# ziwang1121/IEEE

Measured on AMD Instinct MI355X. Metric: 3-modal images/s (train fwd+bwd), higher is better.
Workload: dtype bf16

## Files before the change

### ieee_amd/csrc/bn.hip

```cpp
#include <math.h>
#include <stdlib.h>

#include <hip/hip_ext.h>

#include <algorithm>
#include "common.h"
#include "pool_gather.h"

namespace ieee {

#ifndef IEEE_RED_MAX_BLOCKS
#define IEEE_RED_MAX_BLOCKS 768
#endif
constexpr int RED_MAX_BLOCKS = IEEE_RED_MAX_BLOCKS;

struct RedGeom {
  int M, C;
  int cprw;
  int tx, ty;
  int cblocks;
  int rblocks;
  int rows_per_block;
};

// ... 369 lines not shown
      const float* sp = stats + z * stats_gs + 2 * C + c0;
      load_floats<VEC>(sp, sc);
      load_floats<VEC>(sp + C, sh);
    }
  }
  const T* dd = da + z * gs;
  const T* aa = MASK == 1 ? a + z * gs : nullptr;
  const T* yy = y + z * gs;
  T* oo = dy + z * gs;
  T* go = GOUT ? gout + z * gs : nullptr;
  const int64_t stride = (int64_t)gridDim.x * 256;
  auto finish = [&](int64_t i, const uint4& dv, const uint4& yv, const uint4& av) {
    float d[VEC], v[VEC], m[VEC];
    Vec16<T>::unpack(dv, d);
    Vec16<T>::unpack(yv, v);
    if (MASK == 1) {
      Vec16<T>::unpack(av, m);
#pragma unroll
      for (int e = 0; e < VEC; ++e) d[e] = m[e] > 0.f ? d[e] : 0.f;
    } else if (MASK == 2) {
#pragma unroll
      for (int e = 0; e < VEC; ++e) d[e] = (v[e] * sc[e] + sh[e]) > 0.f ? d[e] : 0.f;
    }
    if (GOUT) *(uint4*)(go + i * VEC) = Vec16<T>::pack(d);
#pragma unroll
    for (int e = 0; e < VEC; ++e) v[e] = k1[e] * d[e] + k2[e] * v[e] + k3[e];
    *(uint4*)(oo + i * VEC) = Vec16<T>::pack(v);
  };
  int64_t i = (int64_t)blockIdx.x * 256 + threadIdx.x;
  if (UNROLL == 2)
    for (; i + stride < total_chunks; i += 2 * stride) {
      const int64_t j = i + stride;
      const uint4 d0 = *(const uint4*)(dd + i * VEC), d1 = *(const uint4*)(dd + j * VEC);
      const uint4 y0 = *(const uint4*)(yy + i * VEC), y1 = *(const uint4*)(yy + j * VEC);
      uint4 a0 = y0, a1 = y1;
      if (MASK == 1) { a0 = *(const uint4*)(aa + i * VEC); a1 = *(const uint4*)(aa + j * VEC); }
      finish(i, d0, y0, a0);
      finish(j, d1, y1, a1);
    }
  for (; i < total_chunks; i += stride) {
    const uint4 d0 = *(const uint4*)(dd + i * VEC);
    const uint4 y0 = *(const uint4*)(yy + i * VEC);
    uint4 a0 = y0;
    if (MASK == 1) a0 = *(const uint4*)(aa + i * VEC);
    finish(i, d0, y0, a0);
  }
}

constexpr double TOT_INV_FWD = 1.0 / 16777216.0;
constexpr double TOT_INV_BWD = 1.0 / 1099511627776.0;
constexpr long long TOT_HALF_RANGE = 1ll << 61;
__device__ __forceinline__ long long tot_abs(long long v) { return v < 0 ? -v : v; }

template <typename T, bool RES, bool BITS>
__global__ __launch_bounds__(256) void bn_apply_totals_kernel(const T* __restrict__ y, const T* __restrict__ residual,
                                                              T* __restrict__ out, const long long* __restrict__ totals,
                                                              const float* __restrict__ gamma, const float* __restrict__ beta,
                                                              int64_t param_gs, float* running_mean, float* running_var,
                                                              int64_t buf_gs, float* __restrict__ stats, int M, float momentum,
                                                              float eps, int64_t total_chunks, int cprw, int C, int64_t gs,
                                                              int relu, uint8_t* __restrict__ relu_bits, double inv_m,
                                                              float unbias, int rep, int64_t rep_stride, int* overflow) {
  constexpr int VEC = 16 / sizeof(T);
  const int z = blockIdx.y;
  uint8_t* bb = BITS ? relu_bits + z * (gs / 8) : nullptr;
  const int c0 = (threadIdx.x & (cprw - 1)) * VEC;
  const T* yy = y + z * gs;
  const T* rr = RES ? residual + z * gs : nullptr;
  const int64_t stride = (int64_t)gridDim.x * 256;
  int64_t i = (int64_t)blockIdx.x * 256 + threadIdx.x;
  uint4 ynext = make_uint4(0, 0, 0, 0), rnext = make_uint4(0, 0, 0, 0);
  if (out != nullptr && i < total_chunks) {
    ynext = *(const uint4*)(yy + i * VEC);
    if (RES) rnext = *(const uint4*)(rr + i * VEC);
  }
  extern __shared__ float tot_lds[];
  float* s_sc = tot_lds;
  float* s_sh = tot_lds + C;
  for (int c = threadIdx.x; c < C; c += 256) {
    long long t1 = 0, t2 = 0;
    for (int r = 0; r < rep; ++r) {
      t1 += totals[r * rep_stride + (int64_t)z * 2 * C + c];
      t2 += totals[r * rep_stride + (int64_t)z * 2 * C + C + c];
    }
    if (blockIdx.x == 0 && overflow != nullptr && (tot_abs(t1) > TOT_HALF_RANGE || tot_abs(t2) > TOT_HALF_RANGE)) *(volatile int*)(overflow + 2) = 1;
    const float ga = gamma[z * param_gs + c], be = beta[z * param_gs + c];
    const double mu = (double)t1 * inv_m;
    double var = (double)t2 * inv_m - mu * mu;
    if (var < 0) var = 0;
    const float mean = (float)mu, varf = (float)var, invstd = rsqrtf(varf + eps);
    const float scv = ga * invstd, shv = be - mean * scv;
    s_sc[c] = scv; s_sh[c] = shv;
    if (blockIdx.x == 0) {
      float* st = stats + (int64_t)z * 4 * C;
      st[c] = mean; st[C + c] = invstd; st[2 * C + c] = scv; st[3 * C + c] = shv;
      if (running_mean != nullptr) {
        float* rm = running_mean + z * buf_gs + c;
        float* rv = running_var + z * buf_gs + c;
        *rm = (1.f - momentum) * *rm + momentum * mean;
        *rv = (1.f - momentum) * *rv + momentum * (varf * unbias);
      }
    }
  }
  __syncthreads();
  float sc[VEC], sh[VEC];
  load_floats<VEC>(s_sc + c0, sc);
  load_floats<VEC>(s_sh + c0, sh);
  if (out == nullptr) return;
  T* oo = out + z * gs;
  for (; i < total_chunks; i += stride) {
    float v[VEC], r[VEC];
    Vec16<T>::unpack(ynext, v);
    if (RES) Vec16<T>::unpack(rnext, r);
    if (i + stride < total_chunks) {
      ynext = *(const uint4*)(yy + (i + stride) * VEC);
      if (RES) rnext = *(const uint4*)(rr + (i + stride) * VEC);
    }
#pragma unroll
    for (int e = 0; e < VEC; ++e) {
      float x = v[e] * sc[e] + sh[e];
      if (RES) x += r[e];
      if (relu) x = fmaxf(x, 0.f);
      v[e] = x;
    }
    const uint4 pv = Vec16<T>::pack(v);
    *(uint4*)(oo + i * VEC) = pv;
    if constexpr (BITS && VEC == 8) {
      Vec16<T>::unpack(pv, v);
      unsigned b = 0;
#pragma unroll
      for (int e = 0; e < VEC; ++e) b |= (v[e] > 0.f ? 1u : 0u) << e;
      bb[i] = (uint8_t)b;
    }
  }
}

template <typename T, int MASK, bool GOUT>
__global__ __launch_bounds__(256) void bn_bwd_apply_totals_kernel(const T* __restrict__ da, const T* __restrict__ a,
                                                                  const T* __restrict__ y, T* __restrict__ dy,
                                                                  T* __restrict__ gout, const long long* __restrict__ totals,
                                                                  const float* __restrict__ gamma, int64_t param_gs,
                                                                  const float* __restrict__ stats, float* dgamma,
                                                                  float* dbeta, int64_t grad_gs, int M, int64_t total_chunks,
                                                                  int cprw, int C, int64_t gs, double inv_m, int rep,
                                                                  int64_t rep_stride, int* overflow) {
  constexpr int VEC = 16 / sizeof(T);
  const int z = blockIdx.y;
  const int c0 = (threadIdx.x & (cprw - 1)) * VEC;
  const float* st = stats + (int64_t)z * 4 * C;
  const T* dd = da + z * gs;
  const T* aa = MASK == 1 ? a + z * gs : nullptr;
  const T* yy = y + z * gs;
  const int64_t stride = (int64_t)gridDim.x * 256;
  int64_t i = (int64_t)blockIdx.x * 256 + threadIdx.x;
  uint4 dnext = make_uint4(0, 0, 0, 0), ynext = dnext, anext = dnext;
  if (i < total_chunks) {
    dnext = *(const uint4*)(dd + i * VEC);
    ynext = *(const uint4*)(yy + i * VEC);
    if (MASK == 1) anext = *(const uint4*)(aa + i * VEC);
  }
  extern __shared__ float tot_lds[];
  float* s_k = tot_lds;
  for (int c = threadIdx.x; c < C; c += 256) {
    long long t1 = 0, t2 = 0;
    for (int r = 0; r < rep; ++r) {
      t1 += totals[r * rep_stride + (int64_t)z * 2 * C + c];
      t2 += totals[r * rep_stride + (int64_t)z * 2 * C + C + c];
    }
    if (blockIdx.x == 0 && overflow != nullptr && (tot_abs(t1) > TOT_HALF_RANGE || tot_abs(t2) > TOT_HALF_RANGE)) *(volatile int*)(overflow + 3) = 1;
// ... 557 lines not shown

namespace ieee {
__global__ void bn_frozen_coef_kernel(const float* __restrict__ stats, int64_t stats_gs, float* __restrict__ coef,
                                      int64_t coef_gs, int C) {
  const int c = blockIdx.x * blockDim.x + threadIdx.x;
  if (c >= C) return;
  float* k = coef + blockIdx.y * coef_gs;
  k[c] = stats[blockIdx.y * stats_gs + 2 * C + c];
  k[C + c] = 0.f;
  k[2 * C + c] = 0.f;
}
}

extern "C" int ieee_bn2d_bwd_frozen(const void* dout, const void* out_mask, const void* y, void* dy, void* g_out, int dtype,
                                    int64_t groups, int64_t M, int64_t C, int64_t act_gs, const float* stats, float* coef,
                                    int mask_from_y, void* done_event, void* stream) {
  IEEE_REQUIRE(dout && y && dy && stats && coef, "bn2d_bwd_frozen: null pointer");
  IEEE_REQUIRE(dtype == IEEE_F32 || dtype == IEEE_BF16, "bn2d_bwd_frozen: bad dtype");
  IEEE_REQUIRE(C % vec_of(dtype) == 0, "bn2d_bwd_frozen: C not a multiple of the vector width");
  hipStream_t st = (hipStream_t)stream;
  bn_frozen_coef_kernel<<<dim3(cdiv(C, 256), (unsigned)groups), 256, 0, st>>>(stats, 4 * C, coef, 3 * C, (int)C);
  IEEE_TRY(launch_status("bn_frozen_coef_kernel"));
  return launch_bwd_apply(dout, out_mask, y, dy, g_out, dtype, groups, M, C, act_gs, stats, coef, mask_from_y, done_event, st);
}

extern "C" int ieee_bn2d_fwd_totals(const void* y, const void* residual, void* out, int dtype, int64_t groups, int64_t M,
                                    int64_t C, int64_t act_gs, const float* gamma, const float* beta, int64_t param_gs,
                                    float* running_mean, float* running_var, int64_t buf_gs, float* stats, const void* totals,
                                    int replicas, float momentum, float eps, int relu, void* relu_bits, int* overflow,
                                    void* stream) {
  IEEE_REQUIRE(replicas >= 1 && replicas <= 64, "bn2d_fwd_totals: 1..64 replicas");
  IEEE_REQUIRE(y && gamma && beta && stats && totals, "bn2d_fwd_totals: null pointer");
  IEEE_REQUIRE(dtype == IEEE_BF16, "bn2d_fwd_totals: bf16 only (the fused statistics exist on the bf16 path)");
  const int cprw = (int)(C / 8);
  IEEE_REQUIRE(C % 8 == 0 && cprw >= 1 && cprw <= 256 && 256 % cprw == 0, "bn2d_fwd_totals: C / 8 must divide 256");
  IEEE_REQUIRE(!relu_bits || (out && act_gs % 8 == 0), "bn2d_fwd_totals: relu_bits needs an output");
  IEEE_REQUIRE((((uintptr_t)totals | (uintptr_t)gamma | (uintptr_t)beta) & 15) == 0 && param_gs % 4 == 0,
               "bn2d_fwd_totals: totals / gamma / beta must be 16-byte aligned (group stride a multiple of 4 floats)");
  hipStream_t st = (hipStream_t)stream;
  const int64_t chunks = M * C / 8;
  dim3 grid(out ? tot_blocks(chunks, groups) : 1, (unsigned)groups);
  const bf16 *yb = (const bf16*)y, *rb = (const bf16*)residual;
  bf16* ob = (bf16*)out;
  uint8_t* bits = (uint8_t*)relu_bits;
#define IEEE_BN_TOT(RES, BITS)                                                                                              \
  bn_apply_totals_kernel<bf16, RES, BITS><<<grid, 256, 2 * C * sizeof(float), st>>>(yb, rb, ob, (const long long*)totals, gamma, beta, param_gs, \
      running_mean, running_var, buf_gs, stats, (int)M, momentum, eps, chunks, cprw, (int)C, act_gs, relu, bits,       \
      TOT_INV_FWD / (double)M, M > 1 ? (float)((double)M / (double)(M - 1)) : 1.0f, replicas, groups * 2 * C, overflow)
  if (residual && bits) IEEE_BN_TOT(true, true);
  else if (residual) IEEE_BN_TOT(true, false);
  else if (bits) IEEE_BN_TOT(false, true);
  else IEEE_BN_TOT(false, false);
#undef IEEE_BN_TOT
  return launch_status("bn_apply_totals_kernel");
}

extern "C" int ieee_bn2d_bwd_totals(const void* dout, const void* out_mask, const void* y, void* dy, void* g_out, int dtype,
                                    int64_t groups, int64_t M, int64_t C, int64_t act_gs, const float* gamma,
                                    int64_t param_gs, const float* stats, float* dgamma, float* dbeta, int64_t grad_gs,
                                    const void* totals, int replicas, int mask_from_y, int* overflow, void* done_event,
                                    void* stream) {
  IEEE_REQUIRE(replicas >= 1 && replicas <= 64, "bn2d_bwd_totals: 1..64 replicas");
  IEEE_REQUIRE(dout && y && dy && gamma && stats && totals, "bn2d_bwd_totals: null pointer");
  IEEE_REQUIRE(dtype == IEEE_BF16, "bn2d_bwd_totals: bf16 only");
  const int cprw = (int)(C / 8);
  IEEE_REQUIRE(C % 8 == 0 && cprw >= 1 && cprw <= 256 && 256 % cprw == 0, "bn2d_bwd_totals: C / 8 must divide 256");
  IEEE_REQUIRE((((uintptr_t)totals | (uintptr_t)gamma | (uintptr_t)stats) & 15) == 0 && param_gs % 4 == 0,
               "bn2d_bwd_totals: totals / gamma / stats must be 16-byte aligned (group stride a multiple of 4 floats)");
  hipStream_t st = (hipStream_t)stream;
  hipEvent_t ev = (hipEvent_t)done_event;
  const int64_t chunks = M * C / 8;
  dim3 grid(tot_blocks(chunks, groups), (unsigned)groups);
  const int variant = (out_mask ? 1 : (mask_from_y ? 2 : 0)) * 2 + (g_out ? 1 : 0);
#define IEEE_BN_BWD_TOT(MASK, GOUT)                                                                                          \
  case MASK * 2 + (GOUT ? 1 : 0):                                                                                            \
    hipExtLaunchKernelGGL((bn_bwd_apply_totals_kernel<bf16, MASK, GOUT>), grid, dim3(256), 3 * C * sizeof(float), st,        \
                          nullptr, ev, 0,                                                                                    \
                          (const bf16*)dout, (const bf16*)out_mask, (const bf16*)y, (bf16*)dy, (bf16*)g_out,                 \
                          (const long long*)totals, gamma, param_gs, stats, dgamma, dbeta, grad_gs, (int)M, chunks, cprw,    \
                          (int)C, act_gs, 1.0 / (double)M, replicas, groups * 2 * C, overflow);                              \
    break;
  switch (variant) {
    IEEE_BN_BWD_TOT(0, false) IEEE_BN_BWD_TOT(0, true) IEEE_BN_BWD_TOT(1, false) IEEE_BN_BWD_TOT(1, true)
    IEEE_BN_BWD_TOT(2, false) IEEE_BN_BWD_TOT(2, true)
  }
#undef IEEE_BN_BWD_TOT
  return launch_status("bn_bwd_apply_totals_kernel");
}

extern "C" int ieee_bn2d_bwd_totals_ds(const void* dout, const void* y, const void* y_ds, void* dy, int dtype, int64_t groups,
                                       int64_t M, int64_t C, int64_t act_gs, const float* gamma, int64_t param_gs,
                                       const float* stats, float* dgamma, float* dbeta, int64_t grad_gs, const void* totals,
                                       int replicas, void* totals_ds, int replicas_ds, int* overflow, void* done_event,
                                       void* stream) {
  IEEE_REQUIRE(replicas >= 1 && replicas <= 64 && replicas_ds >= 1 && replicas_ds <= 64, "bn2d_bwd_totals_ds: 1..64 replicas");
  IEEE_REQUIRE(dout && y && y_ds && dy && gamma && stats && totals && totals_ds, "bn2d_bwd_totals_ds: null pointer");
  IEEE_REQUIRE(dtype == IEEE_BF16, "bn2d_bwd_totals_ds: bf16 only");
  const int cprw = (int)(C / 8);
  IEEE_REQUIRE(C % 8 == 0 && cprw >= 1 && cprw <= 256 && 256 % cprw == 0, "bn2d_bwd_totals_ds: C / 8 must divide 256");
  IEEE_REQUIRE((((uintptr_t)totals | (uintptr_t)gamma | (uintptr_t)stats) & 15) == 0 && param_gs % 4 == 0,
               "bn2d_bwd_totals_ds: totals / gamma / stats must be 16-byte aligned (group stride a multiple of 4 floats)");
  hipStream_t st = (hipStream_t)stream;
  const int64_t chunks = M * C / 8;
  dim3 grid(tot_blocks(chunks, groups), (unsigned)groups);
  const size_t lds = std::max<size_t>(3 * C, 8 * 256) * sizeof(float);
  const float lim2 = nextafterf(4611686018427387904.0f / (float)grid.x, 0.f);
// ... 82 lines not shown
```

### ieee_amd/csrc/net.hip

```cpp
#include <stdio.h>
#include <stdlib.h>
#include <string.h>

#include <map>
#include <string>
#include <vector>

#include "common.h"

namespace {

using namespace ieee;

struct Tensor {
  size_t off = 0;
  int64_t numel = 0;
  int dtype = IEEE_F32;
};

static constexpr int TOT_REP_MAX = 8;
static int totals_tiles() {
  static const int t = getenv("IEEE_BN_TOTALS_TILES") ? atoi(getenv("IEEE_BN_TOTALS_TILES")) : 1024;
  return t;
}
// ... 49 lines not shown
  return m;
}

struct Block {
  int c1, c2, c3, ds;
};

struct Net {
  static constexpr int NGBUF = 15;
  int B, H, W, num_classes, dtype, interaction, attention, using_rem;
  int frozen = 0;
  int parts = 6, rdim = 768, cdim = 128, fdim = 2048, hid = 128;
  float bn_eps = 1e-5f, bn_mom = 0.1f;
  std::vector<std::string> slot_names;
  std::vector<int64_t> slot_off;
  std::vector<int> triples;
  float *params = nullptr, *grads = nullptr, *buffers = nullptr;
  bool bound = false;
  std::vector<ConvUnit> units;
  std::vector<Block> blocks;
  int u_stem = -1, u_one = -1, u_rest = -1;
  int s_ca1, s_ca2, s_rw, s_rg, s_rb, s_rrm, s_rrv, s_rem_param, s_rem_pw, s_rem_pb, s_rem_qw, s_rem_qb;
  int s_fcw[18], s_fcb[18], s_fcg[18], s_fcbe[18], s_fcrm[18], s_fcrv[18], s_clw[18], s_clb[18];
  size_t ws_bytes = 0;
  std::map<std::string, Tensor> tensors;
  Tensor x0, pool, pool_arg, S, gbuf[NGBUF], slab, bnpart, bncoef, bnpart2, bncoef2, packtab, gemm_work;
  static constexpr int RT_SLOTS = 24, RT_MAX = 32;
  Tensor rtab;
  std::vector<ieee_wgrad_reduce_desc> rpend;
  std::vector<ieee_wgrad_reduce_desc> rtab_host[RT_SLOTS];
  const void* rtab_ws[RT_SLOTS] = {};
  ConvUnit reduce_unit;
  size_t tot_begin = 0, tot_end = 0;
  Tensor slab2;
  ieee_wgrad_reduce_desc wpend = {};
  int wflip = 0;
  Tensor wtickets;
  Tensor tickets;
  std::vector<PackDescHost> pack_train, pack_eval;
  int pack_blocks_train = 0, pack_blocks_eval = 0;
  std::vector<PackDescHost> pack_late;
  int pack_late_first = 0, pack_late_unit = 0, pack_blocks_early = 0, pack_blocks_late = 0;
  std::vector<PackDescHost> pack_train_s, pack_late_s;
  int pack_blocks_train_s = 0, pack_late_first_s = 0, pack_blocks_early_s = 0, pack_blocks_late_s = 0;
  const void* shadow = nullptr;
  hipEvent_t pack_ev[2] = {nullptr, nullptr};
  const void* pack_uploaded_ws = nullptr;
  bool fused_bwd_state = false;
  Tensor oflags;
  const void* last_ws = nullptr;
  bool totals_off = false;
  bool bwd_totals_fresh = false;
  bool bwd_totals_state = false;
  bool stem_a_valid = false;
  bool eval_cache_valid = false;
  const void* eval_cache_ws = nullptr;
  hipStream_t side = nullptr;
  hipStream_t side2 = nullptr;
  hipEvent_t branch_ev[16] = {};
  std::vector<hipEvent_t> side_ready;
  hipEvent_t gbuf_read[NGBUF] = {};
  hipEvent_t side_done = nullptr;
  hipEvent_t sync_ev = nullptr;
  bool gbuf_pending[NGBUF] = {};
  uint64_t gbuf_seq[NGBUF] = {}, gbuf_clock = 0;
  int gbuf_evt[NGBUF] = {};
  bool side_dirty = false;
  size_t side_used = 0;
  ~Net() {
    for (hipEvent_t e : ev_pool) (void)hipEventDestroy(e);
    for (hipEvent_t e : side_ready) (void)hipEventDestroy(e);
    for (hipEvent_t e : gbuf_read) if (e) (void)hipEventDestroy(e);
    if (side_done) (void)hipEventDestroy(side_done);
    if (sync_ev) (void)hipEventDestroy(sync_ev);
    for (hipEvent_t e : pack_ev) if (e) (void)hipEventDestroy(e);
    if (side) (void)hipStreamDestroy(side);
    for (hipEvent_t e : branch_ev) if (e) (void)hipEventDestroy(e);
    if (side2) (void)hipStreamDestroy(side2);
  }
  Tensor Gp, avgmax, amax, Hh, Hs, att, Pp, Zg, Zp, glob, part, sv_g, sv_p, rr, part2, fcraw, sv_fc, featcat, fcall,
      logits, featn, norms;
  Tensor dfeatcat, dfcraw, dpart2, dr, dglob, dZp, dZg, dPp, dGp, datt, dHs, dH, davgmax, remwork;
  int esz() const { return dtype == IEEE_BF16 ? 2 : 4; }
  char* tap_base = nullptr;
  size_t tap_bytes = 0, tap_used = 0;
  std::map<std::string, Tensor> taps;
  int profiling = 0;
  std::vector<hipEvent_t> ev_pool;
  std::vector<int> ev_cat;
  std::vector<std::string> ev_name;
  std::vector<const char*> ev_label;
  std::vector<double> ev_flops;
  size_t ev_used = 0;
  double prof_flops[2] = {0, 0};
  int64_t prof_launches[2] = {0, 0};

  int slot3(const std::string& pattern) {
    const int id = (int)slot_names.size();
    triples.push_back(id);
    for (int m = 0; m < 3; ++m) {
      std::string s = pattern;
      const size_t p = s.find("{m}");
      s.replace(p, 3, std::to_string(m));
      slot_names.push_back(s);
    }
    return id;
// ... 277 lines not shown
    Tensor t;
    t.off = n.tap_used; t.numel = numel; t.dtype = dt;
    IEEE_HIP(hipMemcpyAsync(n.tap_base + t.off, p, bytes, hipMemcpyDeviceToDevice, (hipStream_t)st));
    n.taps[name] = t;
    n.tap_used += (bytes + 255) / 256 * 256;
    return IEEE_OK;
  }
  int64_t in_numel(const ConvUnit& u) const { return (int64_t)3 * B * u.Hi * u.Wi * u.Ci; }
  int64_t out_numel(const ConvUnit& u) const { return (int64_t)3 * u.M(B) * u.Co; }
  bool fused_stats = false;
  bool fused_fin = false;
  bool frz(const ConvUnit& u) const { return (n.frozen & u.child) != 0; }
  int totals_rep(const ConvUnit& u) const { return n.totals_off ? 0 : totals_rep_for((u.M(B) + 127) / 128); }
  bool use_totals(const ConvUnit& u) const {
    return n.dtype == IEEE_BF16 && totals_rep(u) > 0 && u.Co % 8 == 0 && 256 % (u.Co / 8) == 0 && u.Co / 8 <= 256 &&
           &u != &n.units[n.u_stem] && ((n.slot_off[u.s_g] | n.slot_off[u.s_b] | gs(u.s_g)) & 3) == 0;
  }
  bool fwd_totals = false;
  int conv(const ConvUnit& u, const void* in, bool want_stats = false) {
    const int64_t ldf = ieee_conv_packed_ld(n.dtype, u.Ci, u.R, u.S);
    fused_stats = want_stats && n.dtype == IEEE_BF16 && !frz(u);
    fwd_totals = fused_stats && use_totals(u);
    static const bool f_fin = getenv("IEEE_BN_FIN_FUSE") && atoi(getenv("IEEE_BN_FIN_FUSE")) != 0;
    fused_fin = f_fin && fused_stats && !fwd_totals && u.M(B) <= ieee_conv2d_fwd_bn_train_max_rows() && u.Ci % 64 == 0 && u.Co % 8 == 0;
    prof_begin(0, u, nullptr, !fused_fin);
    struct G { Run* r; ~G() { r->prof_end(); } } guard{this};
    if (fused_fin)
      return ieee_conv2d_fwd_bn_train(in, P(u.wf), P(u.y), n.dtype, 3, B, u.Hi, u.Wi, u.Ci, u.Co, u.R, u.S, u.stride, u.pad,
                                      (int64_t)B * u.Hi * u.Wi * u.Ci, u.Co * ldf, u.M(B) * u.Co, bnpart_cur, par(u.s_g), par(u.s_b),
                                      gs(u.s_g), buf(u.s_rm), buf(u.s_rv), gs(u.s_rm), F(u.stats), n.bn_mom, n.bn_eps, tickets_cur, st);
    const bool sh = use_shadow && u.shadow_ok;
    const void* wf = sh ? (const void*)((const uint16_t*)n.shadow + n.slot_off[u.s_w]) : P(u.wf);
    return ieee_conv2d_fwd_ex(in, wf, P(u.y), n.dtype, 3, B, u.Hi, u.Wi, u.Ci, u.Co, u.R, u.S, u.stride, u.pad,
                              (int64_t)B * u.Hi * u.Wi * u.Ci, sh ? gs(u.s_w) : u.Co * ldf, u.M(B) * u.Co, fused_stats ? bnpart_cur : nullptr,
                              take_extras(fwd_totals ? P(u.tot_f) : nullptr, (int64_t)2 * u.Co, fwd_totals ? totals_rep(u) : 1), st);
  }
  int bn(const ConvUnit& u, const void* residual, void* out, int relu, int training, void* relu_bits = nullptr) {
    if (frz(u)) training = 0;
    if (training && fwd_totals) {
      fwd_totals = fused_stats = fused_fin = false;
      return ieee_bn2d_fwd_totals(P(u.y), residual, out, n.dtype, 3, u.M(B), u.Co, u.M(B) * u.Co, par(u.s_g), par(u.s_b), gs(u.s_g),
                                  buf(u.s_rm), buf(u.s_rv), gs(u.s_rm), F(u.stats), P(u.tot_f), totals_rep(u), n.bn_mom, n.bn_eps, relu, relu_bits,
                                  oflags_ptr(), st);
    }
    fwd_totals = false;
    const int64_t rb = (training && fused_fin) ? -1 : ((training && fused_stats) ? ieee_conv2d_fwd_stats_rblocks(B, u.Ho, u.Wo) : 0);
    fused_stats = false;
    fused_fin = false;
    if (rb < 0 && out == nullptr) return IEEE_OK;
    return ieee_bn2d_fwd(P(u.y), residual, out, n.dtype, 3, u.M(B), u.Co, u.M(B) * u.Co, par(u.s_g), par(u.s_b),
                         gs(u.s_g), buf(u.s_rm), buf(u.s_rv), gs(u.s_rm), F(u.stats), bnpart_cur, n.bn_mom, n.bn_eps,
                         training, relu, rb, relu_bits, st);
  }
  bool eval_cached = false;
  int conv_bn_eval(const ConvUnit& u, const void* in, const void* residual, void* out, int relu) {
    const int64_t ldf = ieee_conv_packed_ld(n.dtype, u.Ci, u.R, u.S);
    if (!eval_cached)
      IEEE_TRY(ieee_bn2d_fwd(P(u.y), nullptr, nullptr, n.dtype, 3, u.M(B), u.Co, u.M(B) * u.Co, par(u.s_g), par(u.s_b),
                           gs(u.s_g), buf(u.s_rm), buf(u.s_rv), gs(u.s_rm), F(u.stats), bnpart_cur, n.bn_mom, n.bn_eps,
                           0, relu, 0, nullptr, st));
    prof_begin(0, u);
    struct G { Run* r; ~G() { r->prof_end(); } } guard{this};
    return ieee_conv2d_fwd_bn_eval(in, P(u.wf), out, residual, F(u.stats), relu, n.dtype, 3, B, u.Hi, u.Wi, u.Ci, u.Co,
                                   u.R, u.S, u.stride, u.pad, (int64_t)B * u.Hi * u.Wi * u.Ci, u.Co * ldf, u.M(B) * u.Co, st);
  }
  bool& fused_bwd = n.fused_bwd_state;
  hipEvent_t bn_done = nullptr;
  hipEvent_t next_ready_event() {
    if (n.side_used == n.side_ready.size()) {
      hipEvent_t e;
      if (hipEventCreateWithFlags(&e, hipEventDisableTiming) != hipSuccess) return nullptr;
      n.side_ready.push_back(e);
    }
    return n.side_ready[n.side_used++];
  }
  const ConvUnit* ds_pending = nullptr;
  const ConvUnit* ds_totals_ready = nullptr;
  int bn_bwd(const ConvUnit& u, const void* dout, const void* mask, void* dy, void* gout, int mask_from_y = 0,
             float* partial = nullptr, int64_t partial_rb = 0) {
    const int64_t rb = partial ? partial_rb : (fused_bwd ? (u.M(B) + 127) / 128 : 0);
    const bool ds_ready = !partial && ds_totals_ready == &u;
    if (ds_ready) ds_totals_ready = nullptr;
    const bool from_totals = (!partial && fused_bwd && n.bwd_totals_state) || ds_ready;
    const ConvUnit* ds = ds_pending;
    ds_pending = nullptr;
    if (!partial) partial = bnpart_cur;
    fused_bwd = false;
    n.bwd_totals_state = false;
    will_write(dy);
    if (gout) will_write(gout);
    static const bool ride_wanted = !(getenv("IEEE_EVENT_RIDE") && atoi(getenv("IEEE_EVENT_RIDE")) == 0);
    const bool ride = ride_wanted && side_enabled() && ieee_event_ride_selfcheck(st, (void*)n.side) == 0;
    bn_done = ride ? next_ready_event() : nullptr;
    if (frz(u))
      return ieee_bn2d_bwd_frozen(dout, mask, P(u.y), dy, gout, n.dtype, 3, u.M(B), u.Co, u.M(B) * u.Co, F(u.stats), bncoef_cur,
                                  mask_from_y, (void*)bn_done, st);
    if (from_totals && ds != nullptr && mask == nullptr && gout == nullptr && !mask_from_y && use_totals(*ds) && !frz(*ds) && ds->Co == u.Co &&
        ds->M(B) == u.M(B)) {
      ds_totals_ready = ds;
      return ieee_bn2d_bwd_totals_ds(dout, P(u.y), P(ds->y), dy, n.dtype, 3, u.M(B), u.Co, u.M(B) * u.Co, par(u.s_g), gs(u.s_g), F(u.stats),
                                     grd(u.s_g), grd(u.s_b), gs(u.s_g), P(u.tot_b), totals_rep(u), P(ds->tot_b), totals_rep(*ds),
                                     oflags_ptr(), (void*)bn_done, st);
    }
    if (from_totals)
      return ieee_bn2d_bwd_totals(dout, mask, P(u.y), dy, gout, n.dtype, 3, u.M(B), u.Co, u.M(B) * u.Co, par(u.s_g), gs(u.s_g),
                                  F(u.stats), grd(u.s_g), grd(u.s_b), gs(u.s_g), P(u.tot_b), totals_rep(u), mask_from_y, oflags_ptr(),
// ... 317 lines not shown
    const int64_t n_early = use_shadow ? N.pack_late_first_s : N.pack_late_first;
    const int b_train = use_shadow ? N.pack_blocks_train_s : N.pack_blocks_train, b_late = use_shadow ? N.pack_blocks_late_s : N.pack_blocks_late,
              b_early = use_shadow ? N.pack_blocks_early_s : N.pack_blocks_early;
    static const bool pack_async = !(getenv("IEEE_PACK_ASYNC") && atoi(getenv("IEEE_PACK_ASYNC")) == 0);
    if (training && pack_async && side_enabled() && n_late > 0) {
      IEEE_HIP(hipEventRecord(N.pack_ev[0], (hipStream_t)st));
      IEEE_HIP(hipStreamWaitEvent(N.side, N.pack_ev[0], 0));
      IEEE_TRY(ieee_pack_all_weights(N.params, ws, t_late, n_late, b_late, dt, (void*)N.side));
      IEEE_HIP(hipEventRecord(N.pack_ev[1], N.side));
      late_pack_pending = true;
      if (n_early > 0) IEEE_TRY(ieee_pack_all_weights(N.params, ws, t_train, n_early, b_early, dt, st));
    } else if (training)
      IEEE_TRY(ieee_pack_all_weights(N.params, ws, t_train, n_train, b_train, dt, st));
    else if (!(eval_cached = (N.eval_cache_valid && N.eval_cache_ws == (const void*)ws && !N.profiling)))
      IEEE_TRY(ieee_pack_all_weights(N.params, ws, tab_dev, (int64_t)N.pack_eval.size(), N.pack_blocks_eval, dt, st));
    if (training) N.eval_cache_valid = false;
  }
  {
    static const bool f_fin = getenv("IEEE_BN_FIN_FUSE") && atoi(getenv("IEEE_BN_FIN_FUSE")) != 0;
    if (training && f_fin) IEEE_HIP(hipMemsetAsync(P(N.tickets), 0, 512 * 4, (hipStream_t)st));
  }
  if (training && dt == IEEE_BF16 && (totals_tiles() > 0 || wgrad_fold())) {
    IEEE_HIP(hipMemsetAsync(ws + N.tot_begin, 0, N.tot_end - N.tot_begin, (hipStream_t)st));
    N.bwd_totals_fresh = true;
  }
  IEEE_TRY(ieee_nchw_to_nhwc3(xr, xn, xt, P(N.x0), dt, B, 3, N.H, N.W, 4, 3, st));
  const ConvUnit& s = N.units[N.u_stem];
  static const bool fuse_eval = !(getenv("IEEE_EVAL_FUSE") && atoi(getenv("IEEE_EVAL_FUSE")) == 0);
  const bool fe = !training && fuse_eval;
  bool stem_pool_fused = false;
  if (fe) {
    IEEE_TRY(conv_bn_eval(s, P(N.x0), nullptr, P(s.a), 1));
  } else {
    IEEE_TRY(conv(s, P(N.x0), training != 0));
    static const bool fuse_pool = !(getenv("IEEE_STEM_POOL_FUSE") && atoi(getenv("IEEE_STEM_POOL_FUSE")) == 0);
    stem_pool_fused = training && fuse_pool;
    IEEE_TRY(bn(s, nullptr, stem_pool_fused ? nullptr : P(s.a), 1, training));
  }
  N.stem_a_valid = !stem_pool_fused;
  if (stem_pool_fused)
    IEEE_TRY(ieee_bn_relu_maxpool3x3s2_fwd(P(s.y), F(s.stats), P(N.pool), (uint8_t*)P(N.pool_arg), dt, 3, B, s.Ho, s.Wo, s.Co, st));
  else
    IEEE_TRY(ieee_maxpool3x3s2_fwd(P(s.a), P(N.pool), (uint8_t*)P(N.pool_arg), dt, 3, B, s.Ho, s.Wo, s.Co, st));
  const void* x = P(N.pool);
  int ds_slot = 0;
  for (const Block& b : N.blocks) {
    const ConvUnit &c1 = N.units[b.c1], &c2 = N.units[b.c2], &c3 = N.units[b.c3];
    if (late_pack_pending && b.c1 >= N.pack_late_unit) {
      IEEE_HIP(hipStreamWaitEvent((hipStream_t)st, N.pack_ev[1], 0));
      late_pack_pending = false;
    }
    const bool ws_ = training != 0;
    const bool par_ds = b.ds >= 0 && training && branch_enabled(1);
    if (par_ds) {
      const ConvUnit& d = N.units[b.ds];
      BranchScope scope(*this, ds_slot);
      IEEE_TRY(conv(d, x, ws_));
      IEEE_TRY(bn(d, nullptr, P(d.a), 0, training));
    }
    if (fe) {
      IEEE_TRY(conv_bn_eval(c1, x, nullptr, P(c1.a), 1));
      IEEE_TRY(conv_bn_eval(c2, P(c1.a), nullptr, P(c2.a), 1));
      const void* idn = x;
      if (b.ds >= 0) {
        const ConvUnit& d = N.units[b.ds];
        IEEE_TRY(conv_bn_eval(d, x, nullptr, P(d.a), 0));
        idn = P(d.a);
      }
      IEEE_TRY(conv_bn_eval(c3, P(c2.a), idn, P(c3.a), 1));
      x = P(c3.a);
      continue;
    }
    IEEE_TRY(conv(c1, x, ws_));
    IEEE_TRY(bn(c1, nullptr, P(c1.a), 1, training));
    IEEE_TRY(conv(c2, P(c1.a), ws_));
    IEEE_TRY(bn(c2, nullptr, P(c2.a), 1, training));
    const void* identity = x;
    if (b.ds >= 0) {
      const ConvUnit& d = N.units[b.ds];
      if (par_ds) {
        branch_join(ds_slot);
      } else {
        IEEE_TRY(conv(d, x, ws_));
        IEEE_TRY(bn(d, nullptr, P(d.a), 0, training));
      }
      identity = P(d.a);
      ++ds_slot;
    }
    IEEE_TRY(conv(c3, P(c2.a), ws_));
    IEEE_TRY(bn(c3, identity, P(c3.a), 1, training, (training && c3.abits.numel) ? P(c3.abits) : nullptr));
    x = P(c3.a);
  }
  const void* Fm = x;
  const ConvUnit &uo = N.units[N.u_one], &ur = N.units[N.u_rest];
  const int Hh_ = uo.Hi, Ww = uo.Wi, C = N.fdim;
  const int64_t BC = (int64_t)B * C;
  IEEE_TRY(ieee_gpool_sum_others(Fm, N.interaction ? P(N.S) : nullptr, F(N.Gp), dt, B, Hh_, Ww, C, st));
  const int mode = !N.interaction ? 2 : (N.attention ? 0 : 1);
  if (N.interaction) {
    IEEE_TRY(conv(uo, Fm, training != 0));
    if (!eval_cached) IEEE_TRY(bn(uo, nullptr, nullptr, 1, training));
    IEEE_TRY(conv(ur, P(N.S), training != 0));
    if (!eval_cached) IEEE_TRY(bn(ur, nullptr, nullptr, 1, training));
    if (N.attention) {
      IEEE_TRY(ieee_ca_pool(P(ur.y), F(ur.stats), F(N.avgmax), F(N.avgmax) + BC, 2 * BC, (int32_t*)P(N.amax), dt, B, Hh_,
                            Ww, C, st));
      IEEE_TRY(gemm3(F(N.avgmax), 2 * BC, par(N.s_ca1), gs(N.s_ca1), F(N.Hh), 2 * B * N.hid, nullptr, 0, 2 * B, N.hid, C,
                     C, 1, C, 1, N.hid, 1, 0));
      IEEE_TRY(ieee_ca_mix_fwd(F(N.Hh), F(N.Hs), B, N.hid, st));
      IEEE_TRY(gemm3(F(N.Hs), (int64_t)B * N.hid, par(N.s_ca2), gs(N.s_ca2), F(N.att), BC, nullptr, 0, B, C, N.hid,
                     N.hid, 1, N.hid, 1, C, 0, 0));
      IEEE_TRY(ieee_sigmoid_fwd(F(N.att), 3 * BC, st));
    }
    IEEE_TRY(ieee_cim_tail_fwd(P(uo.y), P(ur.y), F(uo.stats), F(ur.stats), F(N.att), F(N.Pp), dt, B, Hh_, Ww, C, N.parts,
                               mode, st));
  } else {
    IEEE_TRY(ieee_cim_tail_fwd(Fm, nullptr, nullptr, nullptr, nullptr, F(N.Pp), dt, B, Hh_, Ww, C, N.parts, 2, st));
  }
  const int R = N.rdim, PB = N.parts * B;
  {
    Set3 g, p;
    set3(g, F(N.Gp), BC, par(N.s_rw), gs(N.s_rw), F(N.Zg), (int64_t)B * R, nullptr, 0, B, R, C, C, 1, C, 1, R, 0, 0);
    set3(p, F(N.Pp), (int64_t)PB * C, par(N.s_rw), gs(N.s_rw), F(N.Zp), (int64_t)PB * R, nullptr, 0, PB, R, C, C, 1, C, 1, R, 0, 0);
    IEEE_TRY(gemm_pair(g.s, p.s));
  }
  {
    const void *x1[3], *x2[3], *ga[3], *be[3];
    void *o1[3], *o2[3], *rm[3], *rv[3], *s1[3], *s2[3];
    for (int m = 0; m < 3; ++m) {
      x1[m] = F(N.Zg) + (int64_t)m * B * R; o1[m] = F(N.glob) + (int64_t)m * B * R;
      x2[m] = F(N.Zp) + (int64_t)m * PB * R; o2[m] = F(N.part) + (int64_t)m * PB * R;
      ga[m] = par(N.s_rg + m); be[m] = par(N.s_rb + m); rm[m] = buf(N.s_rrm + m); rv[m] = buf(N.s_rrv + m);
      s1[m] = F(N.sv_g) + m * 2 * R; s2[m] = F(N.sv_p) + m * 2 * R;
    }
    const int tr_red = (training && !(N.frozen & IEEE_FROZEN_REDUCE)) ? 1 : 0;
    IEEE_TRY(ieee_rowbn_fwd(3, x1, o1, ga, be, rm, rv, s1, B, R, R, R, N.bn_mom, N.bn_eps, tr_red, 1, st));
    IEEE_TRY(ieee_rowbn_fwd(3, x2, o2, ga, be, rm, rv, s2, PB, R, R, R, N.bn_mom, N.bn_eps, tr_red, 1, st));
  }
  const float* p2 = F(N.part);
  if (N.using_rem) {
    IEEE_TRY(gemm3(F(N.glob), (int64_t)B * R, par(N.s_rem_pw), gs(N.s_rem_pw), F(N.rr), (int64_t)B * R, par(N.s_rem_pb),
                   gs(N.s_rem_pb), B, R, R, R, 1, R, 1, R, 0, 0));
    IEEE_TRY(ieee_rem_fwd(F(N.part), F(N.rr), par(N.s_rem_param), gs(N.s_rem_param), F(N.part2), B, N.parts, R, st));
// ... 589 lines not shown
  for (size_t i = 0; i + 1 < n->ev_used; i += 2) {
    float t = 0.f;
    if (hipEventElapsedTime(&t, n->ev_pool[i], n->ev_pool[i + 1]) != hipSuccess) {
      (void)hipGetLastError();
      continue;
    }
    ms[n->ev_cat[i / 2]] += t;
  }
  if (const char* path = getenv("IEEE_PROFILE_DUMP")) {
    if (FILE* f = fopen(path, "w")) {
      fprintf(f, "unit,kind,us,gflop,tflops\n");
      for (size_t i = 0; i + 1 < n->ev_used; i += 2) {
        float t = 0.f;
        (void)hipEventElapsedTime(&t, n->ev_pool[i], n->ev_pool[i + 1]);
        fprintf(f, "%s,%s,%.2f,%.3f,%.1f\n", n->ev_name[i / 2].c_str(), n->ev_label[i / 2], t * 1e3,
                n->ev_flops[i / 2] / 1e9, n->ev_flops[i / 2] / (t * 1e-3) / 1e12);
      }
      fclose(f);
    }
  }
  for (int c = 0; c < 2; ++c) { out6[c * 3 + 0] = ms[c]; out6[c * 3 + 1] = n->prof_flops[c]; out6[c * 3 + 2] = (double)n->prof_launches[c]; }
  return IEEE_OK;
}

extern "C" int ieee_net_debug_taps(void* handle, void* buffer, int64_t bytes) {
  Net* n = as_net(handle);
  IEEE_REQUIRE(n && (buffer == nullptr || bytes > 0), "net_debug_taps: bad arguments");
  n->tap_base = (char*)buffer;
  n->tap_bytes = buffer ? (size_t)bytes : 0;
  n->tap_used = 0;
  n->taps.clear();
  return IEEE_OK;
}

extern "C" int ieee_net_debug_tap(void* handle, const char* name, int64_t* byte_offset, int64_t* numel, int* dtype) {
  Net* n = as_net(handle);
  IEEE_REQUIRE(n && name && byte_offset && numel && dtype, "net_debug_tap: null pointer");
  auto it = n->taps.find(name);
  IEEE_REQUIRE(it != n->taps.end(), "net_debug_tap: no tap named '%s' (set a buffer and run the backward first)", name);
  *byte_offset = (int64_t)it->second.off;
  *numel = it->second.numel;
  *dtype = it->second.dtype;
  return IEEE_OK;
}

extern "C" int ieee_net_tensor(void* handle, const char* name, int64_t* byte_offset, int64_t* numel, int* dtype) {
  Net* n = as_net(handle);
  IEEE_REQUIRE(n && name && byte_offset && numel && dtype, "net_tensor: null pointer");
  auto it = n->tensors.find(name);
  IEEE_REQUIRE(it != n->tensors.end(), "net_tensor: unknown tensor '%s'", name);
  IEEE_REQUIRE(n->stem_a_valid || n->u_stem < 0 || n->units[n->u_stem].name + ".a" != name,
               "net_tensor: '%s' was not produced by the last forward (a training forward pools straight from the stem's conv "
               "output; IEEE_STEM_POOL_FUSE=0 materialises it)", name);
  *byte_offset = (int64_t)it->second.off;
  *numel = it->second.numel;
  *dtype = it->second.dtype;
  return IEEE_OK;
}
```

### include/ieee_amd.h

```cpp
#ifndef IEEE_AMD_H
#define IEEE_AMD_H

#include <stdint.h>

#ifdef __cplusplus
extern "C" {
#endif

#define IEEE_OK 0
#define IEEE_ERR_BAD_ARG (-1)
#define IEEE_ERR_HIP (-2)
#define IEEE_ERR_UNSUPPORTED (-3)
#define IEEE_ERR_NO_VALID_QUERY (-4)

#define IEEE_F32 0
#define IEEE_BF16 1

#define IEEE_MAX_GROUPS 18

const char* ieee_last_error(void);
int ieee_version(void);
int ieee_device_is_gfx950(void);

int ieee_sqeuclid_distmat(const void* q, const void* g, int64_t m, int64_t n, int64_t d, int dtype,
// ... 85 lines not shown
  int32_t block_begin;
  int32_t reserved_;
} ieee_wgrad_reduce_desc;
int ieee_conv2d_wgrad_deferred(const void* dy, const void* x, float* dw_oihw, void* work, int dtype, int64_t groups,
                      int64_t N, int64_t Hi, int64_t Wi, int64_t Ci, int64_t Co, int64_t R, int64_t S,
                      int64_t stride, int64_t pad, int64_t dy_gs, int64_t x_gs, int64_t dw_gs, int accumulate,
                      ieee_wgrad_reduce_desc* reduce, void* stream);
int ieee_wgrad_reduce_batch(const ieee_wgrad_reduce_desc* device_descs, int64_t n, int64_t total_blocks, int64_t groups,
                            void* stream);
int ieee_conv2d_wgrad_chained(const void* dy, const void* x, float* dw_oihw, void* work, int dtype, int64_t groups,
                      int64_t N, int64_t Hi, int64_t Wi, int64_t Ci, int64_t Co, int64_t R, int64_t S,
                      int64_t stride, int64_t pad, int64_t dy_gs, int64_t x_gs, int64_t dw_gs, int accumulate,
                      const ieee_wgrad_reduce_desc* prev, ieee_wgrad_reduce_desc* reduce, void* stream);
int ieee_wgrad_reduce_pending(const ieee_wgrad_reduce_desc* pending, int64_t groups, void* stream);


int64_t ieee_bn_partial_floats(int dtype, int64_t M, int64_t C);
int ieee_bn2d_fwd(const void* y, const void* residual, void* out, int dtype, int64_t groups, int64_t M,
                  int64_t C, int64_t act_gs, const float* gamma, const float* beta, int64_t param_gs,
                  float* running_mean, float* running_var, int64_t buf_gs, float* stats, float* partial,
                  float momentum, float eps, int training, int relu, int64_t stats_rblocks, void* relu_bits,
                  void* stream);
int ieee_bn2d_bwd(const void* dout, const void* out_mask, const void* y, void* dy, void* g_out, int dtype,
                  int64_t groups, int64_t M, int64_t C, int64_t act_gs, const float* gamma, int64_t param_gs,
                  const float* stats, float* dgamma, float* dbeta, int64_t grad_gs, float* partial,
                  float* coef, int accumulate, int mask_from_y, int64_t stats_rblocks, void* stream);
int ieee_bn2d_bwd_ev(const void* dout, const void* out_mask, const void* y, void* dy, void* g_out, int dtype,
                  int64_t groups, int64_t M, int64_t C, int64_t act_gs, const float* gamma, int64_t param_gs,
                  const float* stats, float* dgamma, float* dbeta, int64_t grad_gs, float* partial,
                  float* coef, int accumulate, int mask_from_y, int64_t stats_rblocks, void* done_event, void* stream);
int ieee_conv_next_bn_totals(void* totals, int64_t group_stride, int replicas, int* overflow);
typedef struct ieee_conv_extras {
  void* totals;
  int64_t group_stride;
  int32_t replicas;
  int32_t reserved_;
  int* overflow;
  void* start;
  void* stop;
} ieee_conv_extras;
int ieee_conv2d_fwd_ex(const void* x, const void* w_packed, void* y, int dtype, int64_t groups, int64_t N, int64_t Hi,
                       int64_t Wi, int64_t Ci, int64_t Co, int64_t R, int64_t S, int64_t stride, int64_t pad, int64_t x_gs,
                       int64_t w_gs, int64_t y_gs, float* bn_partial, const ieee_conv_extras* extras, void* stream);
int ieee_conv2d_dgrad_ex(const void* dy, const void* w_packed_d, void* dx, const void* addend, int dtype,
                         int64_t groups, int64_t N, int64_t Hi, int64_t Wi, int64_t Ci, int64_t Co, int64_t R,
                         int64_t S, int64_t stride, int64_t pad, int64_t dy_gs, int64_t w_gs, int64_t dx_gs,
                         float* bn_partial, const void* bn_y, const void* bn_mask, const float* bn_stats,
                         int bn_mask_bits, int addend_stride, const void* bn_y2, float* bn_partial2,
                         const ieee_conv_extras* extras, void* stream);
int ieee_bn2d_fwd_totals(const void* y, const void* residual, void* out, int dtype, int64_t groups, int64_t M,
                         int64_t C, int64_t act_gs, const float* gamma, const float* beta, int64_t param_gs,
                         float* running_mean, float* running_var, int64_t buf_gs, float* stats, const void* totals,
                         int replicas, float momentum, float eps, int relu, void* relu_bits, int* overflow, void* stream);
int ieee_bn2d_bwd_totals(const void* dout, const void* out_mask, const void* y, void* dy, void* g_out, int dtype,
                         int64_t groups, int64_t M, int64_t C, int64_t act_gs, const float* gamma, int64_t param_gs,
                         const float* stats, float* dgamma, float* dbeta, int64_t grad_gs, const void* totals,
                         int replicas, int mask_from_y, int* overflow, void* done_event, void* stream);
int ieee_bn2d_bwd_totals_ds(const void* dout, const void* y, const void* y_ds, void* dy, int dtype, int64_t groups, int64_t M,
                            int64_t C, int64_t act_gs, const float* gamma, int64_t param_gs, const float* stats,
                            float* dgamma, float* dbeta, int64_t grad_gs, const void* totals, int replicas, void* totals_ds,
                            int replicas_ds, int* overflow, void* done_event, void* stream);
int ieee_bn2d_bwd_frozen(const void* dout, const void* out_mask, const void* y, void* dy, void* g_out, int dtype,
                         int64_t groups, int64_t M, int64_t C, int64_t act_gs, const float* stats, float* coef,
                         int mask_from_y, void* done_event, void* stream);
int ieee_event_ride_selfcheck(void* stream_a, void* stream_b);

int ieee_nchw_to_nhwc3(const float* x_rgb, const float* x_ni, const float* x_ti, void* out, int dtype,
                       int64_t B, int64_t C, int64_t H, int64_t W, int64_t Cpad, int64_t pad, void* stream);
int ieee_maxpool3x3s2_fwd(const void* x, void* out, uint8_t* argmax, int dtype, int64_t groups, int64_t B,
                          int64_t Hi, int64_t Wi, int64_t C, void* stream);
int ieee_bn_relu_maxpool3x3s2_fwd(const void* y, const float* stats, void* out, uint8_t* argmax, int dtype, int64_t groups,
                                  int64_t B, int64_t Hi, int64_t Wi, int64_t C, void* stream);

int ieee_maxpool3x3s2_bwd(const void* dout, const uint8_t* argmax, void* dx, int dtype, int64_t groups,
                          int64_t B, int64_t Hi, int64_t Wi, int64_t C, void* stream);

int ieee_bn2d_bwd_pooled(const void* dpool, const uint8_t* argmax, const void* y, void* dy, int dtype,
                         int64_t groups, int64_t B, int64_t Hi, int64_t Wi, int64_t C, const float* gamma,
                         int64_t param_gs, const float* stats, float* dgamma, float* dbeta, int64_t grad_gs,
                         float* partial, float* coef, int accumulate, void* stream);

int ieee_gpool_sum_others(const void* F, void* S, float* Gp, int dtype, int64_t B, int64_t H, int64_t W,
                          int64_t C, void* stream);
int ieee_ca_pool(const void* y2, const float* stats2, float* avg, float* mx, int64_t pool_gs, int32_t* argmax,
                 int dtype, int64_t B, int64_t H, int64_t W, int64_t C, void* stream);
int ieee_cim_tail_fwd(const void* y1, const void* y2, const float* stats1, const float* stats2,
                      const float* att, float* parts_out, int dtype, int64_t B, int64_t H, int64_t W,
                      int64_t C, int64_t parts, int mode, void* stream);
int ieee_cim_tail_bwd_datt(const float* dparts, const void* y2, const float* stats2, float* datt, int dtype,
                           int64_t B, int64_t H, int64_t W, int64_t C, int64_t parts, void* stream);
int ieee_cim_tail_bwd_g(const float* dparts, const void* y1, const void* y2, const float* stats1,
                        const float* stats2, const float* att, const float* davg, const float* dmax,
                        int64_t pool_gs, const int32_t* argmax, void* g1, void* g2, int dtype, int64_t B,
                        int64_t H, int64_t W, int64_t C, int64_t parts, int mode, float* bn_partial1,
                        float* bn_partial2, void* stream);
int ieee_cim_bwd_combine(const void* D1, const void* DS, const float* dG, void* dF, int dtype, int64_t B,
                         int64_t H, int64_t W, int64_t C, int mode, void* stream);

int ieee_sgemm_grouped(int64_t groups, const void* const* A, const void* const* B, void* const* C,
                       const void* const* bias, int64_t M, int64_t N, int64_t K, int64_t sam, int64_t sak,
                       int64_t sbn, int64_t sbk, int64_t ldc, float alpha, int relu, int accumulate,
                       void* stream);
int ieee_sgemm_grouped_ws(int64_t groups, const void* const* A, const void* const* B, void* const* C,
                          const void* const* bias, int64_t M, int64_t N, int64_t K, int64_t sam, int64_t sak,
                          int64_t sbn, int64_t sbk, int64_t ldc, float alpha, int relu, int accumulate, void* work,
                          int64_t work_bytes, void* stream);
// ... 125 lines not shown
```

Before: 4327.

## Fold downsample-branch BatchNorm apply into the block-output residual BN apply

Adds a DS variant of the totals-based BN apply kernel that computes coefficients for both the main conv and the downsample conv. It applies the downsample BN to the raw residual conv output on the fly, with a bf16 round to match the old materialised activation. In bf16 training the network skips the separate downsample BN pass and its activation write/read, and marks the ds '.a' tensor as unavailable. This saves one elementwise kernel launch and a full activation round trip per downsample block, at the cost of an extra stats computation and extra LDS use per block.

After: 4355, median of 6. Within noise of the previous version (+0.6%).

```diff
diff --git a/ieee_amd/csrc/bn.hip b/ieee_amd/csrc/bn.hip
--- a/ieee_amd/csrc/bn.hip
+++ b/ieee_amd/csrc/bn.hip
@@ -445,7 +445,45 @@
 constexpr long long TOT_HALF_RANGE = 1ll << 61;
 __device__ __forceinline__ long long tot_abs(long long v) { return v < 0 ? -v : v; }
 
-template <typename T, bool RES, bool BITS>
+__device__ __forceinline__ void tot_fwd_coef(int c, int z, int C, const long long* __restrict__ totals, int rep, int64_t rep_stride,
+                                             const float* __restrict__ gamma, const float* __restrict__ beta, int64_t param_gs,
+                                             float* running_mean, float* running_var, int64_t buf_gs, float* __restrict__ stats,
+                                             float momentum, float eps, double inv_m, float unbias, int* overflow, bool publish,
+                                             float* s_sc, float* s_sh) {
+  long long t1 = 0, t2 = 0;
+  for (int r = 0; r < rep; ++r) {
+    t1 += totals[r * rep_stride + (int64_t)z * 2 * C + c];
+    t2 += totals[r * rep_stride + (int64_t)z * 2 * C + C + c];
+  }
+  if (publish && overflow != nullptr && (tot_abs(t1) > TOT_HALF_RANGE || tot_abs(t2) > TOT_HALF_RANGE)) *(volatile int*)(overflow + 2) = 1;
+  const float ga = gamma[z * param_gs + c], be = beta[z * param_gs + c];
+  const double mu = (double)t1 * inv_m;
+  double var = (double)t2 * inv_m - mu * mu;
+  if (var < 0) var = 0;
+  const float mean = (float)mu, varf = (float)var, invstd = rsqrtf(varf + eps);
+  const float scv = ga * invstd, shv = be - mean * scv;
+  s_sc[c] = scv; s_sh[c] = shv;
+  if (publish) {
+    float* st = stats + (int64_t)z * 4 * C;
+    st[c] = mean; st[C + c] = invstd; st[2 * C + c] = scv; st[3 * C + c] = shv;
+    if (running_mean != nullptr) {
+      float* rm = running_mean + z * buf_gs + c;
+      float* rv = running_var + z * buf_gs + c;
+      *rm = (1.f - momentum) * *rm + momentum * mean;
+      *rv = (1.f - momentum) * *rv + momentum * (varf * unbias);
+    }
+  }
+}
+
+struct TotDsUnit {
+  const long long* totals;
+  const float *gamma, *beta;
+  float *running_mean, *running_var, *stats;
+  int64_t param_gs, buf_gs;
+  int rep;
+};
+
+template <typename T, bool RES, bool BITS, bool DS = false>
 __global__ __launch_bounds__(256) void bn_apply_totals_kernel(const T* __restrict__ y, const T* __restrict__ residual,
                                                               T* __restrict__ out, const long long* __restrict__ totals,
                                                               const float* __restrict__ gamma, const float* __restrict__ beta,
@@ -453,7 +491,9 @@
                                                               int64_t buf_gs, float* __restrict__ stats, int M, float momentum,
                                                               float eps, int64_t total_chunks, int cprw, int C, int64_t gs,
                                                               int relu, uint8_t* __restrict__ relu_bits, double inv_m,
-                                                              float unbias, int rep, int64_t rep_stride, int* overflow) {
+                                                              float unbias, int rep, int64_t rep_stride, int* overflow,
+                                                              TotDsUnit ds = TotDsUnit{}) {
+  static_assert(!DS || RES, "the folded branch is the residual");
   constexpr int VEC = 16 / sizeof(T);
   const int z = blockIdx.y;
   uint8_t* bb = BITS ? relu_bits + z * (gs / 8) : nullptr;
@@ -471,34 +511,20 @@
   float* s_sc = tot_lds;
   float* s_sh = tot_lds + C;
   for (int c = threadIdx.x; c < C; c += 256) {
-    long long t1 = 0, t2 = 0;
-    for (int r = 0; r < rep; ++r) {
-      t1 += totals[r * rep_stride + (int64_t)z * 2 * C + c];
-      t2 += totals[r * rep_stride + (int64_t)z * 2 * C + C + c];
-    }
-    if (blockIdx.x == 0 && overflow != nullptr && (tot_abs(t1) > TOT_HALF_RANGE || tot_abs(t2) > TOT_HALF_RANGE)) *(volatile int*)(overflow + 2) = 1;
-    const float ga = gamma[z * param_gs + c], be = beta[z * param_gs + c];
-    const double mu = (double)t1 * inv_m;
-    double var = (double)t2 * inv_m - mu * mu;
-    if (var < 0) var = 0;
-    const float mean = (float)mu, varf = (float)var, invstd = rsqrtf(varf + eps);
-    const float scv = ga * invstd, shv = be - mean * scv;
-    s_sc[c] = scv; s_sh[c] = shv;
-    if (blockIdx.x == 0) {
-      float* st = stats + (int64_t)z * 4 * C;
-      st[c] = mean; st[C + c] = invstd; st[2 * C + c] = scv; st[3 * C + c] = shv;
-      if (running_mean != nullptr) {
-        float* rm = running_mean + z * buf_gs + c;
-        float* rv = running_var + z * buf_gs + c;
-        *rm = (1.f - momentum) * *rm + momentum * mean;
-        *rv = (1.f - momentum) * *rv + momentum * (varf * unbias);
-      }
-    }
+    tot_fwd_coef(c, z, C, totals, rep, rep_stride, gamma, beta, param_gs, running_mean, running_var, buf_gs, stats, momentum, eps,
+                 inv_m, unbias, overflow, blockIdx.x == 0, s_sc, s_sh);
+    if constexpr (DS)
+      tot_fwd_coef(c, z, C, ds.totals, ds.rep, rep_stride, ds.gamma, ds.beta, ds.param_gs, ds.running_mean, ds.running_var, ds.buf_gs,
+                   ds.stats, momentum, eps, inv_m, unbias, overflow, blockIdx.x == 0, s_sc + 2 * C, s_sh + 2 * C);
   }
   __syncthreads();
-  float sc[VEC], sh[VEC];
+  float sc[VEC], sh[VEC], scd[DS ? VEC : 1], shd[DS ? VEC : 1];
   load_floats<VEC>(s_sc + c0, sc);
   load_floats<VEC>(s_sh + c0, sh);
+  if constexpr (DS) {
+    load_floats<VEC>(s_sc + 2 * C + c0, scd);
+    load_floats<VEC>(s_sh + 2 * C + c0, shd);
+  }
   if (out == nullptr) return;
   T* oo = out + z * gs;
   for (; i < total_chunks; i += stride) {
@@ -508,6 +534,11 @@
     if (i + stride < total_chunks) {
       ynext = *(const uint4*)(yy + (i + stride) * VEC);
       if (RES) rnext = *(const uint4*)(rr + (i + stride) * VEC);
+    }
+    if constexpr (DS) {
+#pragma unroll
+      for (int e = 0; e < VEC; ++e) r[e] = r[e] * scd[e] + shd[e];
+      Vec16<T>::unpack(Vec16<T>::pack(r), r);
     }
 #pragma unroll
     for (int e = 0; e < VEC; ++e) {
@@ -1171,6 +1202,41 @@
   else if (bits) IEEE_BN_TOT(false, true);
   else IEEE_BN_TOT(false, false);
 #undef IEEE_BN_TOT
+  return launch_status("bn_apply_totals_kernel");
+}
+
+extern "C" int ieee_bn2d_fwd_totals_ds(const void* y, const void* y_ds, void* out, int dtype, int64_t groups, int64_t M, int64_t C,
+                                       int64_t act_gs, const float* gamma, const float* beta, const float* gamma_ds,
+                                       const float* beta_ds, int64_t param_gs, int64_t param_gs_ds, float* running_mean,
+                                       float* running_var, float* running_mean_ds, float* running_var_ds, int64_t buf_gs,
+                                       int64_t buf_gs_ds, float* stats,
+                                       float* stats_ds, const void* totals, int replicas, const void* totals_ds, int replicas_ds,
+                                       float momentum, float eps, int relu, void* relu_bits, int* overflow, void* stream) {
+  IEEE_REQUIRE(replicas >= 1 && replicas <= 64 && replicas_ds >= 1 && replicas_ds <= 64, "bn2d_fwd_totals_ds: 1..64 replicas");
+  IEEE_REQUIRE(y && y_ds && out && gamma && beta && gamma_ds && beta_ds && stats && stats_ds && totals && totals_ds,
+               "bn2d_fwd_totals_ds: null pointer");
+  IEEE_REQUIRE((running_mean_ds != nullptr) == (running_var_ds != nullptr) && (running_mean != nullptr) == (running_var != nullptr),
+               "bn2d_fwd_totals_ds: running mean and variance come together");
+  IEEE_REQUIRE(dtype == IEEE_BF16, "bn2d_fwd_totals_ds: bf16 only");
+  const int cprw = (int)(C / 8);
+  IEEE_REQUIRE(C % 8 == 0 && cprw >= 1 && cprw <= 256 && 256 % cprw == 0, "bn2d_fwd_totals_ds: C / 8 must divide 256");
+  IEEE_REQUIRE(4 * C * sizeof(float) <= 64 * 1024, "bn2d_fwd_totals_ds: C too large for the coefficient tables");
+  IEEE_REQUIRE(!relu_bits || act_gs % 8 == 0, "bn2d_fwd_totals_ds: relu_bits needs a group stride that is a multiple of 8");
+  IEEE_REQUIRE((((uintptr_t)totals | (uintptr_t)totals_ds | (uintptr_t)gamma | (uintptr_t)beta | (uintptr_t)gamma_ds | (uintptr_t)beta_ds) & 15) == 0 &&
+                   param_gs % 4 == 0 && param_gs_ds % 4 == 0,
+               "bn2d_fwd_totals_ds: totals / gamma / beta must be 16-byte aligned (group stride a multiple of 4 floats)");
+  hipStream_t st = (hipStream_t)stream;
+  const int64_t chunks = M * C / 8;
+  dim3 grid(tot_blocks(chunks, groups), (unsigned)groups);
+  const TotDsUnit ds{(const long long*)totals_ds, gamma_ds, beta_ds, running_mean_ds, running_var_ds, stats_ds, param_gs_ds, buf_gs_ds, replicas_ds};
+#define IEEE_BN_TOT_DS(BITS)                                                                                                         \
+  bn_apply_totals_kernel<bf16, true, BITS, true><<<grid, 256, 4 * C * sizeof(float), st>>>(                                           \
+      (const bf16*)y, (const bf16*)y_ds, (bf16*)out, (const long long*)totals, gamma, beta, param_gs, running_mean, running_var,    \
+      buf_gs, stats, (int)M, momentum, eps, chunks, cprw, (int)C, act_gs, relu, (uint8_t*)relu_bits, TOT_INV_FWD / (double)M,        \
+      M > 1 ? (float)((double)M / (double)(M - 1)) : 1.0f, replicas, groups * 2 * C, overflow, ds)
+  if (relu_bits) IEEE_BN_TOT_DS(true);
+  else IEEE_BN_TOT_DS(false);
+#undef IEEE_BN_TOT_DS
   return launch_status("bn_apply_totals_kernel");
 }
 
diff --git a/ieee_amd/csrc/net.hip b/ieee_amd/csrc/net.hip
--- a/ieee_amd/csrc/net.hip
+++ b/ieee_amd/csrc/net.hip
@@ -125,6 +125,7 @@
   bool totals_off = false;
   bool bwd_totals_fresh = false;
   bool bwd_totals_state = false;
+  bool ds_a_valid = true;
   bool stem_a_valid = false;
   bool eval_cache_valid = false;
   const void* eval_cache_ws = nullptr;
@@ -508,6 +509,17 @@
                          gs(u.s_g), buf(u.s_rm), buf(u.s_rv), gs(u.s_rm), F(u.stats), bnpart_cur, n.bn_mom, n.bn_eps,
                          training, relu, rb, relu_bits, st);
   }
+  bool ds_fold(const ConvUnit& u, const ConvUnit& d, int training) const {
+    return training && n.dtype == IEEE_BF16 && !frz(u) && !frz(d) && use_totals(u) && use_totals(d) && d.Co == u.Co && d.M(B) == u.M(B);
+  }
+  int bn_folded(const ConvUnit& u, const ConvUnit& d, void* out, int relu, void* relu_bits) {
+    IEEE_REQUIRE(fwd_totals, "net: folded BatchNorm apply of '%s' without totals from its conv", u.name.c_str());
+    fwd_totals = fused_stats = fused_fin = false;
+    return ieee_bn2d_fwd_totals_ds(P(u.y), P(d.y), out, n.dtype, 3, u.M(B), u.Co, u.M(B) * u.Co, par(u.s_g), par(u.s_b), par(d.s_g), par(d.s_b),
+                                   gs(u.s_g), gs(d.s_g), buf(u.s_rm), buf(u.s_rv), buf(d.s_rm), buf(d.s_rv), gs(u.s_rm), gs(d.s_rm),
+                                   F(u.stats), F(d.stats), P(u.tot_f), totals_rep(u), P(d.tot_f), totals_rep(d), n.bn_mom, n.bn_eps, relu,
+                                   relu_bits, oflags_ptr(), st);
+  }
   bool eval_cached = false;
   int conv_bn_eval(const ConvUnit& u, const void* in, const void* residual, void* out, int relu) {
     const int64_t ldf = ieee_conv_packed_ld(n.dtype, u.Ci, u.R, u.S);
@@ -931,11 +943,12 @@
     }
     const bool ws_ = training != 0;
     const bool par_ds = b.ds >= 0 && training && branch_enabled(1);
+    const bool fold = b.ds >= 0 && ds_fold(c3, N.units[b.ds], training);
     if (par_ds) {
       const ConvUnit& d = N.units[b.ds];
       BranchScope scope(*this, ds_slot);
       IEEE_TRY(conv(d, x, ws_));
-      IEEE_TRY(bn(d, nullptr, P(d.a), 0, training));
+      if (!fold) IEEE_TRY(bn(d, nullptr, P(d.a), 0, training));
     }
     if (fe) {
       IEEE_TRY(conv_bn_eval(c1, x, nullptr, P(c1.a), 1));
@@ -945,6 +958,7 @@
         const ConvUnit& d = N.units[b.ds];
         IEEE_TRY(conv_bn_eval(d, x, nullptr, P(d.a), 0));
         idn = P(d.a);
+        N.ds_a_valid = true;
       }
       IEEE_TRY(conv_bn_eval(c3, P(c2.a), idn, P(c3.a), 1));
       x = P(c3.a);
@@ -961,13 +975,16 @@
         branch_join(ds_slot);
       } else {
         IEEE_TRY(conv(d, x, ws_));
-        IEEE_TRY(bn(d, nullptr, P(d.a), 0, training));
+        if (fold) fwd_totals = fused_stats = fused_fin = false;
+        else IEEE_TRY(bn(d, nullptr, P(d.a), 0, training));
       }
       identity = P(d.a);
+      N.ds_a_valid = !fold;
       ++ds_slot;
     }
     IEEE_TRY(conv(c3, P(c2.a), ws_));
-    IEEE_TRY(bn(c3, identity, P(c3.a), 1, training, (training && c3.abits.numel) ? P(c3.abits) : nullptr));
+    if (fold) IEEE_TRY(bn_folded(c3, N.units[b.ds], P(c3.a), 1, c3.abits.numel ? P(c3.abits) : nullptr));
+    else IEEE_TRY(bn(c3, identity, P(c3.a), 1, training, (training && c3.abits.numel) ? P(c3.abits) : nullptr));
     x = P(c3.a);
   }
   const void* Fm = x;
@@ -1663,6 +1680,11 @@
   IEEE_REQUIRE(n->stem_a_valid || n->u_stem < 0 || n->units[n->u_stem].name + ".a" != name,
                "net_tensor: '%s' was not produced by the last forward (a training forward pools straight from the stem's conv "
                "output; IEEE_STEM_POOL_FUSE=0 materialises it)", name);
+  if (!n->ds_a_valid)
+    for (const Block& b : n->blocks)
+      IEEE_REQUIRE(b.ds < 0 || n->units[b.ds].name + ".a" != name,
+                   "net_tensor: '%s' was not produced by the last forward (a bf16 training forward folds the downsample branch's "
+                   "BatchNorm into the block-output apply; the branch's conv output is '<unit>.y')", name);
   *byte_offset = (int64_t)it->second.off;
   *numel = it->second.numel;
   *dtype = it->second.dtype;
diff --git a/include/ieee_amd.h b/include/ieee_amd.h
--- a/include/ieee_amd.h
+++ b/include/ieee_amd.h
@@ -161,6 +161,13 @@
                          int64_t C, int64_t act_gs, const float* gamma, const float* beta, int64_t param_gs,
                          float* running_mean, float* running_var, int64_t buf_gs, float* stats, const void* totals,
                          int replicas, float momentum, float eps, int relu, void* relu_bits, int* overflow, void* stream);
+int ieee_bn2d_fwd_totals_ds(const void* y, const void* y_ds, void* out, int dtype, int64_t groups, int64_t M, int64_t C,
+                            int64_t act_gs, const float* gamma, const float* beta, const float* gamma_ds, const float* beta_ds,
+                            int64_t param_gs, int64_t param_gs_ds, float* running_mean, float* running_var,
+                            float* running_mean_ds, float* running_var_ds, int64_t buf_gs, int64_t buf_gs_ds, float* stats,
+                            float* stats_ds, const void* totals, int replicas,
+                            const void* totals_ds, int replicas_ds, float momentum, float eps, int relu, void* relu_bits,
+                            int* overflow, void* stream);
 int ieee_bn2d_bwd_totals(const void* dout, const void* out_mask, const void* y, void* dy, void* g_out, int dtype,
                          int64_t groups, int64_t M, int64_t C, int64_t act_gs, const float* gamma, int64_t param_gs,
                          const float* stats, float* dgamma, float* dbeta, int64_t grad_gs, const void* totals,
```
